# BGU-CS-VIL/DPMMSubClusters.jl

Measured on AMD Instinct MI355X. Metric: Gibbs iterations/sec, N=10M D=64 NIW, higher is better.
Workload: dtype f32

## Files before the change

### dpmmsubclusters.jl_amd/binding.py

```python
import ctypes
import os
import subprocess

import numpy as np

_HERE = os.path.dirname(os.path.abspath(__file__))
PRIOR_NIW, PRIOR_MULT = 0, 1
MAX_CLUSTERS = 1024

_c_i64p = ctypes.POINTER(ctypes.c_int64)
_c_f32p = ctypes.POINTER(ctypes.c_float)
_c_f64p = ctypes.POINTER(ctypes.c_double)

ABI = [
    ("dpmm_abi_version", ctypes.c_int, []),
    ("dpmm_create", ctypes.c_int, [ctypes.POINTER(ctypes.c_void_p), ctypes.c_int, ctypes.c_int, ctypes.c_int64, ctypes.c_int64, ctypes.c_int, ctypes.c_uint64]),
    ("dpmm_destroy", ctypes.c_int, [ctypes.c_void_p]),
    ("dpmm_last_error", ctypes.c_char_p, [ctypes.c_void_p]),
    ("dpmm_upload_points", ctypes.c_int, [ctypes.c_void_p, _c_f32p, ctypes.c_int64]),
    ("dpmm_upload_points_device", ctypes.c_int, [ctypes.c_void_p, ctypes.c_void_p, ctypes.c_int64]),
    ("dpmm_upload_points_npy", ctypes.c_int, [ctypes.c_void_p, ctypes.c_void_p, ctypes.c_int, ctypes.c_int64, ctypes.c_int]),
    ("dpmm_init_labels", ctypes.c_int, [ctypes.c_void_p, ctypes.c_int, ctypes.c_uint32]),
    ("dpmm_set_labels", ctypes.c_int, [ctypes.c_void_p, _c_i64p, _c_i64p]),
    ("dpmm_get_labels", ctypes.c_int, [ctypes.c_void_p, _c_i64p, _c_i64p]),
# ... 44 lines not shown
    ("dpmm_smart_assign", ctypes.c_int, [ctypes.c_void_p, ctypes.c_int64, ctypes.c_double, ctypes.c_double]),
    ("dpmm_debug_loglik", ctypes.c_int, [ctypes.c_void_p, _c_f32p]),
    ("dpmm_sync", ctypes.c_int, [ctypes.c_void_p]),
    ("dpmm_stream", ctypes.c_void_p, [ctypes.c_void_p]),
    ("dpmm_last_sweep_parts_ms", ctypes.c_int, [ctypes.c_void_p, _c_f32p]),
    ("dpmm_last_kernel_ms", ctypes.c_int, [ctypes.c_void_p, _c_f32p, _c_f32p]),
    ("dpmm_debug_counters", ctypes.c_int, [ctypes.c_void_p, ctypes.POINTER(ctypes.c_int64), ctypes.c_int]),
    ("dpmm_debug_set_prelaunch_hook", ctypes.c_int, [ctypes.c_void_p, ctypes.c_void_p]),
    ("dpmm_init_labels_from", ctypes.c_int, [ctypes.c_void_p, ctypes.c_int, ctypes.c_int, ctypes.c_uint32]),
    ("dpmm_set_option", ctypes.c_int, [ctypes.c_void_p, ctypes.c_int, ctypes.c_double]),
    ("dpmm_params_staging", ctypes.c_int, [ctypes.c_void_p, ctypes.c_int] + [ctypes.POINTER(ctypes.c_void_p)] * 6),
    ("dpmm_commit_params", ctypes.c_int, [ctypes.c_void_p, ctypes.c_int]),
    ("dpmm_suffstats_host", ctypes.c_int, [ctypes.c_void_p, _c_i64p, ctypes.c_int, ctypes.POINTER(ctypes.c_void_p)]),
    ("dpmm_step_stats", ctypes.c_int, [ctypes.c_void_p, ctypes.c_uint32, ctypes.POINTER(ctypes.c_void_p), ctypes.POINTER(ctypes.c_void_p)]),
    ("dpmm_debug_subloglik", ctypes.c_int, [ctypes.c_void_p, _c_f32p]),
    ("dpmm_debug_ref_bracket", ctypes.c_int, [ctypes.c_void_p, ctypes.c_int64, ctypes.c_float, _c_f32p, _c_f32p]),
    ("dpmm_debug_pair_ball", ctypes.c_int, [ctypes.c_void_p, _c_f32p, _c_f32p]),
    ("dpmm_debug_bracket_big", ctypes.c_int, [ctypes.c_void_p, _c_f32p, ctypes.POINTER(ctypes.c_uint32)]),
    ("dpmm_debug_mult_draws_ahead", ctypes.c_int, [ctypes.c_void_p, ctypes.POINTER(ctypes.c_longlong)]),
    ("dpmm_last_sweep_work", ctypes.c_int, [ctypes.c_void_p, ctypes.POINTER(ctypes.c_uint64)]),
    ("dpmm_comm_use_library", ctypes.c_int, [ctypes.c_char_p]),
    ("dpmm_comm_unique_id", ctypes.c_int, [ctypes.c_void_p]),
    ("dpmm_comm_init", ctypes.c_int, [ctypes.c_void_p, ctypes.c_void_p, ctypes.c_int, ctypes.c_int]),
    ("dpmm_comm_init_host", ctypes.c_int, [ctypes.c_void_p, ctypes.c_int, ctypes.c_int, ctypes.c_void_p, ctypes.c_void_p]),
    ("dpmm_comm_info", ctypes.c_int, [ctypes.c_void_p, _c_i64p]),
    ("dpmm_last_comm_ms", ctypes.c_int, [ctypes.c_void_p, _c_f32p, _c_f32p]),
    ("dpmm_comm_destroy", ctypes.c_int, [ctypes.c_void_p]),
    ("dpmm_comm_allgather_host", ctypes.c_int, [ctypes.c_void_p, ctypes.c_void_p, ctypes.c_int64, ctypes.c_void_p]),
]

HOST_ALLREDUCE_FN = ctypes.CFUNCTYPE(ctypes.c_int, ctypes.c_void_p, ctypes.c_void_p, ctypes.c_int64, ctypes.c_int)

MASTER_NSCALARS = 8
OPT_SCREEN_MARGIN, OPT_TAIL_SCREEN, OPT_PRESCREEN, OPT_ORDERED_SWEEP, OPT_MULT_FORCE_F32, OPT_STATS_ITEMS, OPT_STATS_GROUPS, OPT_TRACE_SLOW, OPT_LOGLIK_REF_CONST, OPT_WAVE_PRIO, OPT_MULT_NO_U8, OPT_SWEEP_GRID, OPT_SWEEP_QUEUE_ROUNDS, OPT_BALL_SCREEN, OPT_KERNEL_TIMING, OPT_STATS_DERIVE, OPT_NOISE_AHEAD, OPT_REF_BRACKET, OPT_SORT_TILE, OPT_ONE_COLLECTIVE, OPT_BF16_SCREENS, OPT_COMM_TIMEOUT_MS, OPT_DIRECTION_SCREEN, _OPT_RESERVED_24, OPT_MULT_DRAWS_AHEAD, OPT_B3_SUBLABELS, OPT_LEAN_TILES, OPT_MASTER_POLL, OPT_CHAIN_FUSION, OPT_LEAN_DIRECTION, OPT_PAIR_BALL = range(1, 32)


class DpmmError(RuntimeError):
    def __init__(self, code, msg):
        super().__init__(f"libdpmmhip error {code}: {msg}")
        self.code = code


def lib_path():
    return os.path.join(_HERE, "lib", "libdpmmhip.so")


def locked_make(args, lock_dir):
    import fcntl
    os.makedirs(lock_dir, exist_ok=True)
    with open(os.path.join(lock_dir, ".build.lock"), "w") as lk:
        fcntl.flock(lk, fcntl.LOCK_EX)
        try:
            subprocess.check_call(args)
        finally:
            fcntl.flock(lk, fcntl.LOCK_UN)


def build_library(force=False):
    args = ["make", "-s", "-C", os.path.join(_HERE, "csrc"), "-j4"]
    if force:
        args.append("-B")
    locked_make(args, os.path.join(_HERE, "lib"))
    return lib_path()


_LIB = None

# ... 482 lines not shown
```

### dpmmsubclusters.jl_amd/csrc/dpmm_api.cpp

```cpp
#include "../../include/dpmm_hip.h"
#include "../../include/dpmm_hip_master.h"
#include "../../include/dpmm_hip_debug.h"

#include <hip/hip_runtime.h>
#include <dlfcn.h>

#include <algorithm>
#include <atomic>
#include <condition_variable>
#include <mutex>
#include <thread>
#include <chrono>
#include <cmath>
#include <cstdio>
#include <cstring>
#include <cstdlib>
#include <ctime>
#include <string>
#include <unordered_map>
#include <vector>

#include "dpmm_kernels.h"

namespace dpmm {
// ... 157 lines not shown
    int32_t *h_list[4] = {nullptr, nullptr, nullptr, nullptr};
    size_t h_list_cap[4] = {0, 0, 0, 0};
    int h_list_next = 0;
    std::vector<int32_t> jobs_shadow, dslots_shadow;
    uint8_t *h_master = nullptr;
    size_t h_master_bytes = 0;
    bool draws_on_device = false;
    unsigned long long *d_work = nullptr;
    int work_waves = 0;
    long long work_launches = 0;
    float opt_margin = 50.f;
    int opt_prio = 1;
    int opt_queue_rounds = -1;
    int opt_ball = 1;
    uint32_t *d_sp_frag = nullptr;
    uint32_t *d_refb_big = nullptr;
    bool have_refb_big = false;
    uint32_t *d_brk_flag = nullptr;
    float *d_brk_aref = nullptr;
    float *d_sp_cons = nullptr;
    uint32_t *h_need = nullptr;
    int opt_direction = -1;
    bool sp_ready = false, sp_regime = false;
    unsigned sp_count = 0;
    bool sp_last = false;
    int sp_K = -1;
    int sp_cooldown = 0;
    int opt_b3 = 1;
    bool have_b3 = false;
    int opt_chain = 0x7fffffff & ~(8 | 32);
    int opt_pair_ball = 1;
    bool have_pb = false;
    int opt_lean_dir = 1;
    int opt_master_poll = 1;
    int opt_lean = 1;
    uint32_t *d_hard = nullptr;
    int hard_flip = 0;
    int perm_nbins = 0;
    uint32_t *h_hard = nullptr;
    int lean_off = 0;
    bool lean_ran = false;
    int lean_backoff = 15;
    int opt_bf16scr = 1;
    int opt_bracket = 1;
    int opt_timing = 0;
    int opt_tail = 1, opt_prescreen = -1, opt_ordered = 1, opt_force_f32 = 0, opt_trace = 0, opt_ref_const = 0;
    int64_t opt_stats_items = 0;
    int opt_stats_groups = 0;
    void *comm = nullptr;
    int rank = 0, world = 1;
    dpmm_host_allreduce_fn host_fn = nullptr;
    void *host_user = nullptr;
    char *h_red = nullptr;
    size_t h_red_bytes = 0;
    hipEvent_t ev_comm[4] = {nullptr, nullptr, nullptr, nullptr};
    bool have_comm_ev[2] = {false, false};
    int64_t comm_bytes[2] = {0, 0};
    int64_t comm_calls = 0;
    int comm_timeout_ms = 1800000;
    bool coll_pending = false;
    bool abort_reported = false;
    std::thread *watchdog = nullptr;
    std::mutex wd_mu;
    std::condition_variable wd_cv;
    bool wd_stop = false;
    std::atomic<int64_t> wd_wait_since{0};
// ... 868 lines not shown
            a.prio = c->opt_prio;
            a.queue_rounds = c->opt_queue_rounds;
        }
#ifdef DPMM_STAMPS
        if (!g_dbg) { hipMalloc(&g_dbg, sizeof(unsigned long long) * 16 * 4 * 4096); hipMemset(g_dbg, 0, sizeof(unsigned long long) * 16 * 4 * 4096); }
        a.dbg = g_dbg;
#endif
        const bool b3 = c->NB == 4 && c->have_b3 && c->opt_b3 && !table && !c->predictive && a.tail != nullptr;
        if (b3) {
            const bool lean_ok = c->opt_lean != 0 && c->opt_bracket && a.use_prev && a.screen_margin > 0.f && !final_argmax && a.lam == nullptr && c->K > 1 && c->d_hard &&
                                 !(c->opt_lean_dir == 0 && c->sp_regime && c->opt_direction != 0 && c->sp_ready);
            const int64_t nwt = (c->n + 63) / 64;
            if (lean_ok && c->lean_off == 0 && c->lean_ran) {
                if ((int64_t)c->h_hard[0] * 10 > nwt * 3) { c->lean_off = c->lean_backoff; c->lean_backoff = std::min(2 * c->lean_backoff + 1, 1023); }
                else c->lean_backoff = 15;
                c->lean_ran = false;
            }
            const bool use_lean = lean_ok && c->lean_off == 0;
            if (lean_ok && c->lean_off > 0) { c->lean_off -= 1; c->h_hard[0] = 0; }
            const uint32_t *list = nullptr;
            const bool parts = (c->opt_timing & 8) != 0 && (c->opt_timing & 1) != 0;
            if (parts && !c->ev_part[0]) for (auto &e : c->ev_part) HIPCHK(c, hipEventCreate(&e));
            if (use_lean) {
                const size_t hw = hard_list_words(c->n);
                uint32_t *mine = c->d_hard + (size_t)c->hard_flip * hw, *other = c->d_hard + (size_t)(c->hard_flip ^ 1) * hw;
                c->hard_flip ^= 1;
                c->lean_ran = true;
                uint32_t *need2 = a.need ? c->h_need + 8 * (size_t)c->sweep_grid_max : nullptr;
                const bool al = a.order != nullptr && c->perm_nbins > 0 && c->perm_nbins <= NIW_LEAN_MAX_BINS;
                uint32_t *need3 = a.need ? c->h_need + 12 * (size_t)c->sweep_grid_max : nullptr;
                NiwSweepArgs al_args = a;
                if (!c->opt_lean_dir) { al_args.sp_frag = nullptr; al_args.sp_cons = nullptr; }
                if (c->have_pb && c->opt_pair_ball && al_args.ball) al_args.ball |= 2;
                HIPCHK(c, launch_niw_lean(al_args, mine, need2, other, al ? c->sb.bin_start : nullptr, al ? c->perm_nbins : 0, need3, c->sweep_grid, c->stream));
                if (parts) HIPCHK(c, hipEventRecord(c->ev_part[0], c->stream));
                list = mine;
            }
            a.bf16scr |= 4;
            a.tdf = reinterpret_cast<const float *>(list);
            const float *mdist_kept = a.mdist;
            if (list) a.mdist = reinterpret_cast<const float *>(c->h_hard);
            HIPCHK(c, launch_niw_sweep(c->NB, a, c->sweep_grid, c->stream));
            a.mdist = mdist_kept;
            if (parts) HIPCHK(c, hipEventRecord(c->ev_part[1], c->stream));
            c->have_parts = parts ? (use_lean ? 2 : 1) : 0;
            a.bf16scr &= 3;
            a.tdf = nullptr;
            if (!list) HIPCHK(c, launch_niw_sub(a, nullptr, nullptr, c->sweep_grid, c->stream));
        } else {
            HIPCHK(c, launch_niw_sweep(c->NB, a, c->sweep_grid, c->stream));
            if (!table) c->have_parts = 0;
        }
    } else {
        MultSweepArgs a{};
        a.X = c->dX; a.ldx = c->ldx; a.n = c->n; a.first_index = c->first; a.D = c->D; a.K = c->K;
        a.logp = c->d_Rp; a.cst = c->d_cst;
        a.scratch = table ? table : c->d_scratch;
        a.scratch_stride = table ? table_stride : c->scratch_stride;
        a.scratch_by_tile = table ? 1 : 0;
        a.labels_only = table ? 1 : 0;
        a.bins = c->dbins; a.seed = c->seed; a.epoch = epoch; a.final_argmax = final_argmax;
        a.use_prev = c->have_labels ? 1 : 0;
        a.order = (!table && c->have_perm && c->opt_ordered) ? c->sb.perm : nullptr;
        a.order_total = c->sb.perm_total;
        if (c->x_u8) HIPCHK(c, launch_mult_sweep_u8(a, c->dX8, c->ld8, c->d_Lp16, c->sweep_grid, c->stream));
        else if (c->x_bf16_exact) HIPCHK(c, launch_mult_sweep_bf16(a, c->d_Lp16, c->sweep_grid, c->stream));
        else {
// ... 1286 lines not shown
}
#endif

void *dpmm_stream(dpmm_ctx *c) { return c ? (void *)c->stream : nullptr; }

int dpmm_set_option(dpmm_ctx *c, int option, double value) {
    if (!c) return DPMM_EINVAL;
    switch (option) {
        case DPMM_OPT_SCREEN_MARGIN: if (!(value >= 0)) return fail(c, DPMM_EINVAL, "margin < 0"); c->opt_margin = (float)value; return DPMM_OK;
        case DPMM_OPT_TAIL_SCREEN: c->opt_tail = value != 0; return DPMM_OK;
        case DPMM_OPT_PRESCREEN: c->opt_prescreen = value < 0 ? -1 : (value != 0); return DPMM_OK;
        case DPMM_OPT_ORDERED_SWEEP: c->opt_ordered = value != 0; return DPMM_OK;
        case DPMM_OPT_MULT_FORCE_F32:
            if (c->have_points) return fail(c, DPMM_ESTATE, "DPMM_OPT_MULT_FORCE_F32 must be set before the points are uploaded");
            c->opt_force_f32 = value != 0; return DPMM_OK;
        case DPMM_OPT_STATS_ITEMS:
            if (c->Kcap > 0) return fail(c, DPMM_ESTATE, "DPMM_OPT_STATS_ITEMS must be set before the first parameters / K");
            if (value >= 1) c->chunk = (int)std::max<int64_t>((c->prior == DPMM_PRIOR_NIW && c->D <= 64) ? 32 : 256, ((c->n + (int64_t)value - 1) / (int64_t)value + 3) / 4 * 4);
            return DPMM_OK;
        case DPMM_OPT_STATS_GROUPS: c->opt_stats_groups = value > 0 ? (int)value : 0; return DPMM_OK;
        case DPMM_OPT_TRACE_SLOW: c->opt_trace = value != 0; return DPMM_OK;
        case DPMM_OPT_LOGLIK_REF_CONST: c->opt_ref_const = value != 0; return DPMM_OK;
        case DPMM_OPT_WAVE_PRIO: c->opt_prio = value != 0; return DPMM_OK;
        case DPMM_OPT_MULT_DRAWS_AHEAD: c->opt_mult_draws_ahead = value != 0; c->mspec_valid = false; return DPMM_OK;
        case DPMM_OPT_SWEEP_QUEUE_ROUNDS: c->opt_queue_rounds = value < 0 ? -1 : (int)value; return DPMM_OK;
        case DPMM_OPT_BALL_SCREEN: c->opt_ball = value != 0; return DPMM_OK;
        case DPMM_OPT_STATS_DERIVE: c->opt_derive = value != 0; c->cache_force = true; return DPMM_OK;
        case DPMM_OPT_NOISE_AHEAD: c->opt_noise_ahead = value < 0 ? -1 : (value != 0); return DPMM_OK;
        case DPMM_OPT_REF_BRACKET: c->opt_bracket = value != 0; return DPMM_OK;
        case DPMM_OPT_COMM_TIMEOUT_MS: c->comm_timeout_ms = value > 0 ? (int)std::min(value, 2.0e9) : 0; return DPMM_OK;
        case DPMM_OPT_BF16_SCREENS: c->opt_bf16scr = value != 0; return DPMM_OK;
        case DPMM_OPT_MASTER_POLL: c->opt_master_poll = value != 0; return DPMM_OK;
        case DPMM_OPT_PAIR_BALL: c->opt_pair_ball = value != 0; if (!c->opt_pair_ball) c->have_pb = false; return DPMM_OK;
        case DPMM_OPT_LEAN_DIRECTION: c->opt_lean_dir = value != 0; c->lean_off = 0; c->lean_backoff = 15; c->lean_ran = false; return DPMM_OK;
        case DPMM_OPT_CHAIN_FUSION: c->opt_chain = value < 0 ? (0x7fffffff & ~(8 | 32)) : (int)value; return DPMM_OK;
        case DPMM_OPT_LEAN_TILES: c->opt_lean = value != 0; c->lean_off = 0; c->lean_backoff = 15; c->lean_ran = false; return DPMM_OK;
        case DPMM_OPT_B3_SUBLABELS: c->opt_b3 = value != 0; if (!c->opt_b3) c->have_b3 = false; return DPMM_OK;
        case DPMM_OPT_DIRECTION_SCREEN:
            c->opt_direction = value < 0 ? -1 : (value != 0);
            if (c->opt_direction == 0) { c->sp_ready = false; c->sp_regime = false; }
            return DPMM_OK;
        case DPMM_OPT_ONE_COLLECTIVE: c->opt_one_collective = value < 0 ? -1 : (value != 0); return DPMM_OK;
        case DPMM_OPT_SORT_TILE: {
            const int t = (int)value;
            if (t != SORT_TILE && t != SORT_TILE_SMALL) return fail(c, DPMM_EINVAL, "DPMM_OPT_SORT_TILE: 512 or 2048");
            if (t < c->sort_tile_min) {
                if (c->n > 16000000) return fail(c, DPMM_ELIMIT, "DPMM_OPT_SORT_TILE: 512-point tiles are limited to shards of 16e6 points");
                HIPCHK(c, hipSetDevice(c->device));
                HIPCHK(c, sync_stream(c, c->stream));
                const int nt = (int)((c->n + t - 1) / t);
                const size_t nbmax = 2 * DPMM_MAX_CLUSTERS;
                int32_t *th = nullptr, *tc = nullptr, *tsp = nullptr;
                HIPCHK(c, hipMalloc(&th, sizeof(int32_t) * nbmax * (size_t)std::max(1, nt)));
                if (hipMalloc(&tc, sizeof(int32_t) * nbmax * (size_t)std::max(1, nt)) != hipSuccess) { hipFree(th); return fail(c, DPMM_EHIP, "DPMM_OPT_SORT_TILE: out of device memory for the 512-point tile tables"); }
                if (hipMalloc(&tsp, sizeof(int32_t) * (size_t)STEP_SPEC_MAX_BINS * (size_t)std::max(1, nt)) != hipSuccess) { hipFree(th); hipFree(tc); return fail(c, DPMM_EHIP, "DPMM_OPT_SORT_TILE: out of device memory for the 512-point tile tables"); }
                hipFree(c->sb.tile_hist); hipFree(c->sb.tile_cnt); hipFree(c->sb.tile_spec);
                c->sb.tile_hist = th; c->sb.tile_cnt = tc; c->sb.tile_spec = tsp;
                c->nt_sort = nt; c->sort_tile_min = t;
            }
            c->sb.tile = t; return DPMM_OK;
        }
        case DPMM_OPT_KERNEL_TIMING:
            c->opt_timing = (int)value & 15;
            if (!(c->opt_timing & 1)) c->have_sweep_ev = false;
            if (!(c->opt_timing & 2)) c->have_stats_ev = false;
            if (!(c->opt_timing & 4)) c->have_comm_ev[0] = c->have_comm_ev[1] = false;
// ... 302 lines not shown
```

### dpmmsubclusters.jl_amd/csrc/dpmm_kernels.h

```cpp
#pragma once
#include <hip/hip_runtime.h>
#include <stdint.h>

#define DPMM_MAX_CLUSTERS_K 1024

namespace dpmm {


constexpr int DPMM_WORK_QUEUES = 8;
constexpr int DPMM_WORK_SLOTS = 8 + 16 * DPMM_WORK_QUEUES;
constexpr int DPMM_WORK_PER_WAVE = 8;
constexpr int REFB_FRAGS = 6, REFB_WORDS = REFB_FRAGS * 256;
constexpr int B3_WORDS = 3 * REFB_WORDS;
constexpr int B3_DVEC = 64;

struct NiwSweepArgs {
    const float *X;
    int64_t ldx;
    int64_t n;
    int64_t first_index;
    int64_t ntiles;
    int K;
    const float *Rp;
    const float *mup;
// ... 19 lines not shown
    const float *mdist;
    int screen_lds;
    int use_prev;
    int lds_rows;
    const uint32_t *sp_frag;
    const float *sp_cons;
    uint32_t *need;
    unsigned long long *dbg;
    int queue_rounds;
    int prio;
    unsigned long long *work;
};

int niw_tile_points(int NB);
int niw_occupancy(int NB);
hipError_t launch_niw_sweep(int NB, const NiwSweepArgs &a, int grid, hipStream_t s);
hipError_t launch_niw_refb_debug(const NiwSweepArgs &a, int k, float c_override, float *qhi_out, float *q_out, hipStream_t s);
hipError_t launch_niw_screen_prep(const float *R, const float *mu, int D, int K, float *lam, float *dist, const int32_t *slot, hipStream_t s);
hipError_t launch_niw_pack(const float *R, const float *mu, float *Rp, float *mup, int D, int NB, int nmat, float *tail, const float *cst,
                           const int32_t *slot, float *cst_out, unsigned long long *work, hipStream_t s);
constexpr int SP_MAXK = 64, SP_FRAG_WORDS = 4 * 2 * 256, SP_CONS_FLOATS = 3 * 64;
inline size_t niw_refb_big_words(int NB) { size_t c = 0; for (int bi = 0; bi < NB; ++bi) c += NB / 2 - bi / 2; return c * 256; }
hipError_t launch_niw_refb_big(const float *Rp, int NB, int K, uint32_t *out, hipStream_t s);
hipError_t launch_niw_bracket_big(int NB, const NiwSweepArgs &a, const uint32_t *refb, uint32_t *tile_flag, float *aref, hipStream_t s);
hipError_t launch_niw_b3_pack(const float *Rp, const float *mup, int K, float *tail, int what, hipStream_t s);
constexpr int PB_MAXK = 256;
inline size_t niw_pair_ball_floats(size_t K) { return K <= (size_t)PB_MAXK ? K * K + K : 0; }
inline size_t niw_pair_ball_offset(size_t K) { return 32 * ((K + 1) >> 1) + 16 * K + (size_t)REFB_WORDS * K + 3 * K * (size_t)B3_WORDS + 3 * K * (size_t)B3_DVEC; }
inline size_t niw_tail_floats(size_t cap) {
    return 16 * (cap + 2) + 16 * cap + (size_t)REFB_WORDS * cap + 3 * cap * (size_t)B3_WORDS + 3 * cap * (size_t)B3_DVEC + niw_pair_ball_floats(cap < (size_t)PB_MAXK ? cap : (size_t)PB_MAXK);
}
hipError_t launch_niw_b3_debug(const NiwSweepArgs &a, float *out, hipStream_t s);
hipError_t launch_niw_sub(const NiwSweepArgs &a, const uint32_t *list, uint32_t *count_out, int grid, hipStream_t s);
constexpr int NIW_LEAN_MAX_BINS = 256;
hipError_t launch_niw_lean(const NiwSweepArgs &a, uint32_t *list, uint32_t *need2, uint32_t *other_list, const int32_t *bin_start, int nbins, uint32_t *need3, int grid, hipStream_t s);
hipError_t launch_niw_direction(const float *Rp, const float *mup, const float *cst, int D, int K, uint32_t *frag, float *cons, hipStream_t s);

struct MultSweepArgs {
    const float *X;
    int64_t ldx;
    int64_t n;
    int64_t first_index;
    int D;
    int K;
    const float *logp;
    const float *cst;
    float *scratch;
    int64_t scratch_stride;
    int scratch_by_tile;
    int labels_only;
    int32_t *bins;
    uint64_t seed;
    uint32_t epoch;
    int final_argmax;
    int use_prev;
    const int32_t *order;
    const int32_t *order_total;
};
hipError_t launch_mult_sweep(const MultSweepArgs &a, int grid, hipStream_t s);
hipError_t launch_mult_pack(const float *logp, float *Lp, int rows, int64_t ldx, hipStream_t s);
int mult_tile_points();
hipError_t launch_bf16_exact_check(const float *X, int64_t nwords, int *d_flag, hipStream_t s);
size_t mult_pack_bf16_words(int rows, int64_t ldx);
hipError_t launch_mult_pack_bf16(const float *logp, uint32_t *Lp16, int rows, int64_t ldx, hipStream_t s);
hipError_t launch_mult_sweep_bf16(const MultSweepArgs &a, const uint32_t *Lp16, int grid, hipStream_t s);
hipError_t launch_u8_convert(const float *X, int64_t ldx, int D, int64_t n, uint8_t *X8, int64_t ld8, int *d_flag, hipStream_t s);
size_t mult_pack_u8_words(int rows, int64_t ld8);
hipError_t launch_mult_pack_u8(const float *logp, uint32_t *Lp8, int rows, int64_t ldx, int64_t ld8, hipStream_t s);
// ... 142 lines not shown
```

### dpmmsubclusters.jl_amd/csrc/niw_lean.hip

```cpp
#include "dpmm_device.h"
#include "dpmm_kernels.h"
#include "niw_device.h"
#include "niw_b3.h"

namespace dpmm {

__global__ __launch_bounds__(256) void niw_b3_pack_kernel(const float *__restrict__ Rp, const float *__restrict__ mup, float *__restrict__ tail, int K, int y0) {
    constexpr int NP = 10;
    uint32_t *img = const_cast<uint32_t *>(b3_images(tail, K));
    float *dvec = const_cast<float *>(b3_offsets(tail, K));
    const int k = blockIdx.x >> 1, j = 3 * k + 1 + (blockIdx.x & 1);
    const float *Rj = Rp + (size_t)j * NP * 256;
    auto elem = [&](int row, int col) -> float {
        const int bi = row >> 4, t = col >> 4;
        if (t < bi) return 0.f;
        const int pair = pair_base<4>(bi) + (t - bi);
        const int ln = (row & 15) + 16 * ((col & 15) >> 2);
        return Rj[(size_t)pair * 256 + ln * 4 + (col & 3)];
    };
    const int yy = (int)blockIdx.y + y0;
    if (yy == 4) {
        if (blockIdx.x & 1) return;
        const float *Rk = Rp + (size_t)(3 * k) * NP * 256;
        auto elemR = [&](int row, int col) -> float {
// ... 145 lines not shown
#pragma unroll
            for (int sl = 0; sl < 2; ++sl) {
                const int f = bi == 0 ? sl : (bi == 1 ? 2 + sl : (sl == 1 ? bi + 2 : -1));
                if (f < 0) continue;
                const u32x4_t aa = a[f] & absm;
#pragma unroll
                for (int h = 0; h < 2; ++h) {
                    const u32x4_t zb = Z.p[n0 + h][sl][0];
                    y[h] = __builtin_amdgcn_mfma_f32_16x16x32_bf16(__builtin_bit_cast(bf16x8_t, a[f]), __builtin_bit_cast(bf16x8_t, zb), y[h], 0, 0, 0);
                    e[h] = __builtin_amdgcn_mfma_f32_16x16x32_bf16(__builtin_bit_cast(bf16x8_t, aa), __builtin_bit_cast(bf16x8_t, zb & absm), e[h], 0, 0, 0);
                }
            }
#pragma unroll
            for (int h = 0; h < 2; ++h)
#pragma unroll
                for (int r = 0; r < 4; ++r) {
                    const float t = __builtin_fmaf(REFB_C, e[h][r], fabsf(y[h][r]));
                    part[h] = __builtin_fmaf(t, t, part[h]);
                }
        }
#pragma unroll
        for (int h = 0; h < 2; ++h) {
            const f32x4 tot = __builtin_amdgcn_mfma_f32_16x16x4f32(1.0f, part[h], (f32x4){0.f, 0.f, 0.f, 0.f}, 0, 0, 0);
            qhi[n0 + h] = __builtin_fmaf(tot[0], 1.0001f, 1e-20f);
        }
    }
}

#ifdef DPMM_STAMPS
#define LSTAMP(var) unsigned long long var; do { __builtin_amdgcn_sched_barrier(0); asm volatile("s_memtime %0\n\ts_waitcnt lgkmcnt(0)" : "=s"(var) :: "memory"); __builtin_amdgcn_sched_barrier(0); } while (0)
#else
#define LSTAMP(var)
#endif
template <bool DIR>
__device__ __forceinline__ void niw_lean_body(NiwSweepArgs A, uint32_t *__restrict__ list, uint32_t *__restrict__ need2, uint32_t *__restrict__ other_list,
                                              const int32_t *__restrict__ bin_start, int nbins, uint32_t *__restrict__ need3) {
    if (other_list && blockIdx.x == 0 && threadIdx.x == 0) other_list[0] = 0u;
#ifdef DPMM_STAMPS
    unsigned long long T_x = 0, T_conv = 0, T_br = 0, T_scr = 0, T_u = 0, T_p2 = 0, T_tot = 0; int ntl = 0;
#endif
    const int lane = threadIdx.x & 63, ci = lane & 15, g = lane >> 4;
    const bool use_order = A.order != nullptr && *A.order_total == (int32_t)A.n;
    const int K = A.K;
    const int wave_id = (int)blockIdx.x * 4 + (threadIdx.x >> 6), nwaves = (int)gridDim.x * 4;
    unsigned nw_easy = 0, nw_br = 0, nw_tail = 0, nw_bb = 0;
    const bool use_dir = DIR && A.sp_frag != nullptr && A.sp_cons != nullptr && A.bf16scr && K >= 3 && K <= SP_MAXK;
    const bool dir_first = use_dir && (A.bf16scr & 2) != 0;
    unsigned nw_sp = 0, nw_cand = 0, nw_dcand = 0, nw_dexcl = 0, nw_ctiles = 0;
    constexpr int BALL_LDS_K = 256;
    __shared__ __attribute__((aligned(16))) float ball_lds[BALL_LDS_K * 16];
    const bool ball_in_lds = A.ball && K <= BALL_LDS_K;
    __shared__ float pb_s[PB_MAXK];
    const bool use_pb = !DIR && (A.ball & 2) != 0 && ball_in_lds && K <= PB_MAXK;
    const float *pb_d = pair_ball_table(A.tail, K);
    if (use_pb)
        for (int e = threadIdx.x; e < K; e += 256) pb_s[e] = pb_d[(size_t)K * K + e];
    if (ball_in_lds) {
        const float *src = ball_records(A.tail, K);
        for (int e = threadIdx.x; e < 16 * K; e += 256) ball_lds[e] = src[e];
    }
    constexpr int MAXB = NIW_LEAN_MAX_BINS;
    __shared__ int tstart_s[MAXB + 2], bstart_s[MAXB + 2], wsum_s[4];
    const bool aligned = bin_start != nullptr && use_order && nbins >= 1 && nbins <= MAXB && bin_start[nbins] == (int32_t)A.n;
    const int nb = aligned ? nbins : 1;
    {
        const int tid = threadIdx.x;
        int c = 0;
        if (tid < nb) {
            const int s0 = aligned ? bin_start[tid] : 0, s1 = aligned ? bin_start[tid + 1] : (int)A.n;
            c = (s1 - s0 + 63) >> 6; bstart_s[tid] = s0;
        }
        if (tid == 0) bstart_s[nb] = (int)A.n;
        int inc = c;
#pragma unroll
        for (int off = 1; off < 64; off <<= 1) { const int v = __shfl_up(inc, off); if (lane >= off) inc += v; }
        if (lane == 63) wsum_s[tid >> 6] = inc;
        __syncthreads();
        const int w = tid >> 6;
        inc += (w > 0 ? wsum_s[0] : 0) + (w > 1 ? wsum_s[1] : 0) + (w > 2 ? wsum_s[2] : 0);
        tstart_s[tid + 1] = inc;
        if (tid == 0) tstart_s[0] = 0;
    }
    __syncthreads();
    const int ntiles_all = __builtin_amdgcn_readfirstlane(tstart_s[nb]);
    int bptr = 0;
    auto span_of = [&](int t, int &p0, int &cn) {
        p0 = 0; cn = 0;
        if (t >= ntiles_all) return;
        while (t >= __builtin_amdgcn_readfirstlane(tstart_s[bptr + 1])) ++bptr;
        p0 = __builtin_amdgcn_readfirstlane(bstart_s[bptr]) + 64 * (t - __builtin_amdgcn_readfirstlane(tstart_s[bptr]));
        const int e = __builtin_amdgcn_readfirstlane(bstart_s[bptr + 1]) - p0;
        cn = e < 64 ? e : 64;
    };
    auto index_at = [&](int p0, int cn) -> int { return lane < cn ? (use_order ? A.order[p0 + lane] : p0 + lane) : -1; };
    int c_p0, c_cn, n_p0, n_cn;
    span_of(wave_id, c_p0, c_cn);
    span_of(wave_id + nwaves, n_p0, n_cn);
    int nx_p = index_at(c_p0, c_cn);
    auto label_of = [&](int bin) -> int { const int pv = bin >= 0 ? (bin >> 1) : -1; return (unsigned)pv < (unsigned)K ? pv : -1; };
    int nx_prev = label_of(nx_p >= 0 ? A.bins[nx_p] : -1);
    for (int tile = wave_id; tile < ntiles_all; tile += nwaves) {
        const bool valid = lane < c_cn;
        const int myp32 = nx_p;
        LSTAMP(s0);
#ifdef DPMM_STAMPS
        unsigned long long s1 = s0, s2 = s0, s3 = s0, s4 = s0, s5 = s0;
#endif
        const int pf_p = index_at(n_p0, n_cn);
        int pf_bin = -1;
        bool bin_asked = false;
        const int prev = nx_prev;
        const unsigned long long pm = __ballot(prev >= 0);
        bool hard = pm == 0ull;
        int k0 = 0;
        if (!hard) {
            k0 = __builtin_amdgcn_readfirstlane(__shfl(prev, __ffsll((long long)pm) - 1));
            hard = __ballot(valid && prev != k0) != 0ull;
        }
        B3Z Z;
        B3Head H;
        float u_sub = 0.f;
        if (!hard) {
            f32x4 xt = (f32x4){0.f, 0.f, 0.f, 0.f};
            f32x4 x3[4];
            float nz[4] = {0.f, 0.f, 0.f, 0.f};
            u32x4_t abr[6];
            {
                f32x4 x[4][4], mk[4];
                gather_x64(A.X, A.ldx, myp32, ci, g, x);
                b3_mean(A.mup, k0, g, mk);
                {
                    const u32x4_t *F = reinterpret_cast<const u32x4_t *>(refb_records(A.tail, K) + (size_t)k0 * REFB_WORDS) + (unsigned)lane;
#pragma unroll
                    for (int f = 0; f < 6; ++f) abr[f] = F[64 * f];
// ... 102 lines not shown
                    const int pr = (base + sh) >> 1;
                    pend &= ~(3ull << sh);
                    ++nw_tail;
                    cand &= ~((unsigned long long)tail_pair_far(tail_load_pair(A.tail, pr), xt, my_thr) << sh);
                }
                if constexpr (DIR) { if (use_dir && !dir_first) { tile_cand = (unsigned)__builtin_popcountll(cand); direction(); } }
                if (A.bf16scr) {
                    const u32x4_t *Rb0 = reinterpret_cast<const u32x4_t *>(refb_records(A.tail, K));
                    while (cand) {
                        const int k = base + __builtin_ctzll(cand);
                        const u32x4_t a5 = Rb0[(size_t)k * (REFB_WORDS / 4) + 64 * 5 + lane];
                        const f32x4 m4 = *reinterpret_cast<const f32x4 *>(A.mup + (size_t)(3 * k) * 64 + 48 + 4 * g);
                        ++nw_bb;
                        if (!bf16_bottom_excludes<4>(a5, x3, m4, A.cst[3 * k], thrb)) break;
                        cand &= cand - 1ull;
                    }
                }
                hard = cand != 0ull;
                if constexpr (DIR) { if (use_dir && !hard) { nw_cand += tile_cand; nw_sp += tile_sp; nw_dcand += tile_dc; nw_dexcl += tile_dx; ++nw_ctiles; } }
            }
        }
#ifdef DPMM_STAMPS
        { LSTAMP(t4); s4 = t4; }
#endif
        if (!hard) {
            H = b3_head(A.tail, A.cst, K, k0, lane, g);
        }
#ifdef DPMM_STAMPS
        { LSTAMP(t5); s5 = t5; }
#endif
        if (hard) {
            if (lane == 0) { const uint32_t at = atomicAdd(&list[0], 1u); list[1 + 2 * at] = (uint32_t)c_p0; list[2 + 2 * at] = (uint32_t)c_cn; }
            if (!bin_asked && lane < n_cn) pf_bin = A.bins[pf_p];
        } else {
            float bl, br;
            b3_eval(A.tail, K, k0, Z, H, lane, g, bl, br);
            if (valid) A.bins[myp32] = 2 * k0 + draw2(bl, br, u_sub);
            ++nw_easy;
        }
        nx_p = pf_p; nx_prev = label_of(pf_bin);
        asm volatile("" : "+v"(nx_prev));
        c_p0 = n_p0; c_cn = n_cn;
        span_of(tile + 2 * nwaves, n_p0, n_cn);
#ifdef DPMM_STAMPS
        { LSTAMP(s6); T_x += s1 - s0; T_conv += s2 - s1; T_br += s3 - s2; T_scr += s4 - s3; T_u += s5 - s4; T_p2 += s6 - s5; T_tot += s6 - s0; ++ntl; }
#endif
    }
#ifdef DPMM_STAMPS
    if (A.dbg && lane == 0) {
        unsigned long long *d = A.dbg + (size_t)(8192 + wave_id) * 16;
        d[0] = T_x; d[1] = T_conv; d[2] = T_br; d[3] = T_scr; d[4] = T_u; d[5] = T_p2; d[6] = 0; d[7] = T_tot; d[8] = ntl;
    }
#endif
    if (A.work && lane == 0) {
        unsigned long long *slot = A.work + DPMM_WORK_SLOTS + (size_t)wave_id * DPMM_WORK_PER_WAVE;
        slot[0] += nw_easy; slot[3] += nw_tail; slot[4] += nw_br; slot[5] += nw_bb; slot[7] += ((unsigned long long)(2 * nw_easy) << 32) + nw_sp;
    }
    if (need2 && lane == 0) need2[wave_id] = use_dir ? 0u : (nw_easy < 65535u ? nw_easy : 65535u);
    if (need3 && lane == 0) {
        uint32_t word = 0u, yield = 0u;
        if (use_dir) {
            word = ((nw_cand < 65535u ? nw_cand : 65535u) << 16) | (nw_ctiles < 32767u ? nw_ctiles : 32767u) | (dir_first ? 0x8000u : 0u);
            yield = ((nw_dexcl < 65535u ? nw_dexcl : 65535u) << 16) | (nw_dcand < 65535u ? nw_dcand : 65535u);
        }
        need3[2 * wave_id] = word; need3[2 * wave_id + 1] = yield;
    }
}
__global__ __launch_bounds__(256, 2) void niw_lean_kernel(NiwSweepArgs A, uint32_t *__restrict__ list, uint32_t *__restrict__ need2, uint32_t *__restrict__ other_list,
                                                         const int32_t *__restrict__ bin_start, int nbins, uint32_t *__restrict__ need3) {
    niw_lean_body<false>(A, list, need2, other_list, bin_start, nbins, need3);
}
__global__ __launch_bounds__(256, 2) void niw_lean_kernel_dir(NiwSweepArgs A, uint32_t *__restrict__ list, uint32_t *__restrict__ need2, uint32_t *__restrict__ other_list,
                                                             const int32_t *__restrict__ bin_start, int nbins, uint32_t *__restrict__ need3) {
    niw_lean_body<true>(A, list, need2, other_list, bin_start, nbins, need3);
}
hipError_t launch_niw_lean(const NiwSweepArgs &a, uint32_t *list, uint32_t *need2, uint32_t *other_list, const int32_t *bin_start, int nbins, uint32_t *need3, int grid, hipStream_t s) {
    if (!a.tail || a.n <= 0 || !list) return hipErrorInvalidValue;
    if (nbins > NIW_LEAN_MAX_BINS) { bin_start = nullptr; nbins = 0; }
    if (a.sp_frag && a.sp_cons && a.bf16scr && a.K >= 3 && a.K <= SP_MAXK) DPMM_LAUNCH(niw_lean_kernel_dir, dim3(grid), dim3(256), 0, s, a, list, need2, other_list, bin_start, nbins, need3);
    else DPMM_LAUNCH(niw_lean_kernel, dim3(grid), dim3(256), 0, s, a, list, need2, other_list, bin_start, nbins, need3);
    return hipGetLastError();
}

}
```

### include/dpmm_hip.h

```cpp
#ifndef DPMM_HIP_H
#define DPMM_HIP_H

#include <stddef.h>
#include <stdint.h>

#ifdef __cplusplus
extern "C" {
#endif

#define DPMM_ABI_VERSION 3

typedef struct dpmm_ctx dpmm_ctx;

enum { DPMM_PRIOR_NIW = 0, DPMM_PRIOR_MULT = 1 };

enum {
    DPMM_OK = 0,
    DPMM_EINVAL = -1,
    DPMM_ENODEVICE = -2,
    DPMM_EHIP = -3,
    DPMM_ESTATE = -4,
    DPMM_ELIMIT = -5,
    DPMM_ECOMM = -6
};

enum {
    DPMM_OPT_SCREEN_MARGIN = 1,
    DPMM_OPT_TAIL_SCREEN = 2,
    DPMM_OPT_PRESCREEN = 3,
    DPMM_OPT_ORDERED_SWEEP = 4,
    DPMM_OPT_MULT_FORCE_F32 = 5,
    DPMM_OPT_STATS_ITEMS = 6,
    DPMM_OPT_STATS_GROUPS = 7,
    DPMM_OPT_TRACE_SLOW = 8,
    DPMM_OPT_LOGLIK_REF_CONST = 9,
    DPMM_OPT_MULT_NO_U8 = 11,
    DPMM_OPT_SWEEP_GRID = 12,
    DPMM_OPT_SWEEP_QUEUE_ROUNDS = 13,
    DPMM_OPT_BALL_SCREEN = 14,
    DPMM_OPT_STATS_DERIVE = 16,
    DPMM_OPT_NOISE_AHEAD = 17,
    DPMM_OPT_REF_BRACKET = 18,
    DPMM_OPT_SORT_TILE = 19,
    DPMM_OPT_COMM_TIMEOUT_MS = 22,
    DPMM_OPT_B3_SUBLABELS = 26,
    DPMM_OPT_LEAN_TILES = 27,
    DPMM_OPT_MASTER_POLL = 28,
    DPMM_OPT_CHAIN_FUSION = 29,
    DPMM_OPT_LEAN_DIRECTION = 30,
    DPMM_OPT_PAIR_BALL = 31,
    DPMM_OPT_MULT_DRAWS_AHEAD = 25,
    DPMM_OPT_DIRECTION_SCREEN = 23,
    DPMM_OPT_BF16_SCREENS = 21,
    DPMM_OPT_ONE_COLLECTIVE = 20,
    DPMM_OPT_KERNEL_TIMING = 15,
    DPMM_OPT_WAVE_PRIO = 10
};

#define DPMM_MAX_CLUSTERS 1024
#define DPMM_MAX_DIM_NIW 256

int dpmm_abi_version(void);

int dpmm_create(dpmm_ctx **ctx, int prior_kind, int D, int64_t n_local, int64_t first_index,
                int device, uint64_t seed);
int dpmm_destroy(dpmm_ctx *ctx);
const char *dpmm_last_error(const dpmm_ctx *ctx);

int dpmm_upload_points(dpmm_ctx *ctx, const float *X, int64_t ldx);
int dpmm_upload_points_device(dpmm_ctx *ctx, const float *dX, int64_t ldx);
int dpmm_upload_points_npy(dpmm_ctx *ctx, const void *rows, int is_f64, int64_t ld, int nan_to_zero);

int dpmm_init_labels(dpmm_ctx *ctx, int init_clusters, uint32_t epoch);
int dpmm_init_labels_from(dpmm_ctx *ctx, int init_clusters, int first_label, uint32_t epoch);
int dpmm_set_option(dpmm_ctx *ctx, int option, double value);
int dpmm_set_labels(dpmm_ctx *ctx, const int64_t *labels, const int64_t *sub_labels);
int dpmm_get_labels(dpmm_ctx *ctx, int64_t *labels, int64_t *sub_labels);

int dpmm_set_params_niw(dpmm_ctx *ctx, int K, const float *mu, const float *inv_sigma, const float *logdet,
                        const float *lr_weights, const float *weights);
int dpmm_set_params_niw_chol(dpmm_ctx *ctx, int K, const float *mu, const float *R, const float *logdet,
                             const float *lr_weights, const float *weights);
int dpmm_set_params_mult(dpmm_ctx *ctx, int K, const float *logp, const float *lr_weights, const float *weights);
// ... 57 lines not shown
```

Baseline: 696.2.

## Pair waves in 512-thread lean blocks with staggered start and token-gated b3 eval

Adds a paired variant of the lean NIW sweep kernel in which each 512-thread block hosts two groups of four waves. The second group runs at raised priority, waits for its partner to finish a tile before starting, and both groups take turns through a shared-memory token around the b3_eval section. The goal is to stagger phases so one wave's compute overlaps its partner's memory latency and they don't contend for the same unit. It is on by default for the non-direction path (pairing=1), while the direction kernel needs pairing=2. Bounded spin-polls with s_sleep add latency and can stall if the pairing is imbalanced.

Measured after the change: 705.3 (median of 6 runs). 1.01x the previous value.

```diff
diff --git a/dpmmsubclusters.jl_amd/binding.py b/dpmmsubclusters.jl_amd/binding.py
--- a/dpmmsubclusters.jl_amd/binding.py
+++ b/dpmmsubclusters.jl_amd/binding.py
@@ -100,7 +100,7 @@
 HOST_ALLREDUCE_FN = ctypes.CFUNCTYPE(ctypes.c_int, ctypes.c_void_p, ctypes.c_void_p, ctypes.c_int64, ctypes.c_int)
 
 MASTER_NSCALARS = 8
-OPT_SCREEN_MARGIN, OPT_TAIL_SCREEN, OPT_PRESCREEN, OPT_ORDERED_SWEEP, OPT_MULT_FORCE_F32, OPT_STATS_ITEMS, OPT_STATS_GROUPS, OPT_TRACE_SLOW, OPT_LOGLIK_REF_CONST, OPT_WAVE_PRIO, OPT_MULT_NO_U8, OPT_SWEEP_GRID, OPT_SWEEP_QUEUE_ROUNDS, OPT_BALL_SCREEN, OPT_KERNEL_TIMING, OPT_STATS_DERIVE, OPT_NOISE_AHEAD, OPT_REF_BRACKET, OPT_SORT_TILE, OPT_ONE_COLLECTIVE, OPT_BF16_SCREENS, OPT_COMM_TIMEOUT_MS, OPT_DIRECTION_SCREEN, _OPT_RESERVED_24, OPT_MULT_DRAWS_AHEAD, OPT_B3_SUBLABELS, OPT_LEAN_TILES, OPT_MASTER_POLL, OPT_CHAIN_FUSION, OPT_LEAN_DIRECTION, OPT_PAIR_BALL = range(1, 32)
+OPT_SCREEN_MARGIN, OPT_TAIL_SCREEN, OPT_PRESCREEN, OPT_ORDERED_SWEEP, OPT_MULT_FORCE_F32, OPT_STATS_ITEMS, OPT_STATS_GROUPS, OPT_TRACE_SLOW, OPT_LOGLIK_REF_CONST, OPT_WAVE_PRIO, OPT_MULT_NO_U8, OPT_SWEEP_GRID, OPT_SWEEP_QUEUE_ROUNDS, OPT_BALL_SCREEN, OPT_KERNEL_TIMING, OPT_STATS_DERIVE, OPT_NOISE_AHEAD, OPT_REF_BRACKET, OPT_SORT_TILE, OPT_ONE_COLLECTIVE, OPT_BF16_SCREENS, OPT_COMM_TIMEOUT_MS, OPT_DIRECTION_SCREEN, _OPT_RESERVED_24, OPT_MULT_DRAWS_AHEAD, OPT_B3_SUBLABELS, OPT_LEAN_TILES, OPT_MASTER_POLL, OPT_CHAIN_FUSION, OPT_LEAN_DIRECTION, OPT_PAIR_BALL, OPT_LEAN_PAIRING = range(1, 33)
 
 
 class DpmmError(RuntimeError):
diff --git a/dpmmsubclusters.jl_amd/csrc/dpmm_api.cpp b/dpmmsubclusters.jl_amd/csrc/dpmm_api.cpp
--- a/dpmmsubclusters.jl_amd/csrc/dpmm_api.cpp
+++ b/dpmmsubclusters.jl_amd/csrc/dpmm_api.cpp
@@ -213,6 +213,7 @@
     int opt_pair_ball = 1;
     bool have_pb = false;
     int opt_lean_dir = 1;
+    int opt_lean_pair = DPMM_LEAN_PAIRING_DEFAULT;
     int opt_master_poll = 1;
     int opt_lean = 1;
     uint32_t *d_hard = nullptr;
@@ -1147,7 +1148,7 @@
                 NiwSweepArgs al_args = a;
                 if (!c->opt_lean_dir) { al_args.sp_frag = nullptr; al_args.sp_cons = nullptr; }
                 if (c->have_pb && c->opt_pair_ball && al_args.ball) al_args.ball |= 2;
-                HIPCHK(c, launch_niw_lean(al_args, mine, need2, other, al ? c->sb.bin_start : nullptr, al ? c->perm_nbins : 0, need3, c->sweep_grid, c->stream));
+                HIPCHK(c, launch_niw_lean(al_args, mine, need2, other, al ? c->sb.bin_start : nullptr, al ? c->perm_nbins : 0, need3, c->sweep_grid, c->opt_lean_pair, c->stream));
                 if (parts) HIPCHK(c, hipEventRecord(c->ev_part[0], c->stream));
                 list = mine;
             }
@@ -2500,6 +2501,7 @@
         case DPMM_OPT_BF16_SCREENS: c->opt_bf16scr = value != 0; return DPMM_OK;
         case DPMM_OPT_MASTER_POLL: c->opt_master_poll = value != 0; return DPMM_OK;
         case DPMM_OPT_PAIR_BALL: c->opt_pair_ball = value != 0; if (!c->opt_pair_ball) c->have_pb = false; return DPMM_OK;
+        case DPMM_OPT_LEAN_PAIRING: c->opt_lean_pair = value < 0 ? DPMM_LEAN_PAIRING_DEFAULT : std::min((int)value, 2); return DPMM_OK;
         case DPMM_OPT_LEAN_DIRECTION: c->opt_lean_dir = value != 0; c->lean_off = 0; c->lean_backoff = 15; c->lean_ran = false; return DPMM_OK;
         case DPMM_OPT_CHAIN_FUSION: c->opt_chain = value < 0 ? (0x7fffffff & ~(8 | 32)) : (int)value; return DPMM_OK;
         case DPMM_OPT_LEAN_TILES: c->opt_lean = value != 0; c->lean_off = 0; c->lean_backoff = 15; c->lean_ran = false; return DPMM_OK;
diff --git a/dpmmsubclusters.jl_amd/csrc/dpmm_kernels.h b/dpmmsubclusters.jl_amd/csrc/dpmm_kernels.h
--- a/dpmmsubclusters.jl_amd/csrc/dpmm_kernels.h
+++ b/dpmmsubclusters.jl_amd/csrc/dpmm_kernels.h
@@ -75,8 +75,9 @@
 }
 hipError_t launch_niw_b3_debug(const NiwSweepArgs &a, float *out, hipStream_t s);
 hipError_t launch_niw_sub(const NiwSweepArgs &a, const uint32_t *list, uint32_t *count_out, int grid, hipStream_t s);
+constexpr int DPMM_LEAN_PAIRING_DEFAULT = 1;
 constexpr int NIW_LEAN_MAX_BINS = 256;
-hipError_t launch_niw_lean(const NiwSweepArgs &a, uint32_t *list, uint32_t *need2, uint32_t *other_list, const int32_t *bin_start, int nbins, uint32_t *need3, int grid, hipStream_t s);
+hipError_t launch_niw_lean(const NiwSweepArgs &a, uint32_t *list, uint32_t *need2, uint32_t *other_list, const int32_t *bin_start, int nbins, uint32_t *need3, int grid, int pair, hipStream_t s);
 hipError_t launch_niw_direction(const float *Rp, const float *mup, const float *cst, int D, int K, uint32_t *frag, float *cons, hipStream_t s);
 
 struct MultSweepArgs {
diff --git a/dpmmsubclusters.jl_amd/csrc/niw_lean.hip b/dpmmsubclusters.jl_amd/csrc/niw_lean.hip
--- a/dpmmsubclusters.jl_amd/csrc/niw_lean.hip
+++ b/dpmmsubclusters.jl_amd/csrc/niw_lean.hip
@@ -201,9 +201,13 @@
 #else
 #define LSTAMP(var)
 #endif
-template <bool DIR>
+constexpr int LEAN_STAGGER_POLLS = 192, LEAN_TOKEN_POLLS = 48;
+__device__ __forceinline__ int lean_pair_peek(int *w) { return __hip_atomic_load(w, __ATOMIC_RELAXED, __HIP_MEMORY_SCOPE_WORKGROUP); }
+__device__ __forceinline__ void lean_pair_post(int *w, int v) { __hip_atomic_store(w, v, __ATOMIC_RELAXED, __HIP_MEMORY_SCOPE_WORKGROUP); }
+template <bool DIR, bool PAIR>
 __device__ __forceinline__ void niw_lean_body(NiwSweepArgs A, uint32_t *__restrict__ list, uint32_t *__restrict__ need2, uint32_t *__restrict__ other_list,
-                                              const int32_t *__restrict__ bin_start, int nbins, uint32_t *__restrict__ need3) {
+                                              const int32_t *__restrict__ bin_start, int nbins, uint32_t *__restrict__ need3, int pair_nwaves = 0) {
+    constexpr int NT = PAIR ? 512 : 256, NWV = NT / 64;
     if (other_list && blockIdx.x == 0 && threadIdx.x == 0) other_list[0] = 0u;
 #ifdef DPMM_STAMPS
     unsigned long long T_x = 0, T_conv = 0, T_br = 0, T_scr = 0, T_u = 0, T_p2 = 0, T_tot = 0; int ntl = 0;
@@ -211,7 +215,15 @@
     const int lane = threadIdx.x & 63, ci = lane & 15, g = lane >> 4;
     const bool use_order = A.order != nullptr && *A.order_total == (int32_t)A.n;
     const int K = A.K;
-    const int wave_id = (int)blockIdx.x * 4 + (threadIdx.x >> 6), nwaves = (int)gridDim.x * 4;
+    const int wv = __builtin_amdgcn_readfirstlane((int)(threadIdx.x >> 6));
+    const int wave_id = (int)blockIdx.x * NWV + wv, nwaves = PAIR ? pair_nwaves : (int)gridDim.x * 4;
+    const bool has_slot = !PAIR || wave_id < nwaves;
+    __shared__ int pair_s[PAIR ? 16 : 1];
+    const bool younger = PAIR && wv >= 4;
+    if constexpr (PAIR) {
+        if (threadIdx.x < 16) pair_s[threadIdx.x] = 0;
+        if (younger) __builtin_amdgcn_s_setprio(1);
+    }
     unsigned nw_easy = 0, nw_br = 0, nw_tail = 0, nw_bb = 0;
     const bool use_dir = DIR && A.sp_frag != nullptr && A.sp_cons != nullptr && A.bf16scr && K >= 3 && K <= SP_MAXK;
     const bool dir_first = use_dir && (A.bf16scr & 2) != 0;
@@ -223,13 +235,13 @@
     const bool use_pb = !DIR && (A.ball & 2) != 0 && ball_in_lds && K <= PB_MAXK;
     const float *pb_d = pair_ball_table(A.tail, K);
     if (use_pb)
-        for (int e = threadIdx.x; e < K; e += 256) pb_s[e] = pb_d[(size_t)K * K + e];
+        for (int e = threadIdx.x; e < K; e += NT) pb_s[e] = pb_d[(size_t)K * K + e];
     if (ball_in_lds) {
         const float *src = ball_records(A.tail, K);
-        for (int e = threadIdx.x; e < 16 * K; e += 256) ball_lds[e] = src[e];
+        for (int e = threadIdx.x; e < 16 * K; e += NT) ball_lds[e] = src[e];
     }
     constexpr int MAXB = NIW_LEAN_MAX_BINS;
-    __shared__ int tstart_s[MAXB + 2], bstart_s[MAXB + 2], wsum_s[4];
+    __shared__ int tstart_s[MAXB + 2], bstart_s[MAXB + 2], wsum_s[NWV];
     const bool aligned = bin_start != nullptr && use_order && nbins >= 1 && nbins <= MAXB && bin_start[nbins] == (int32_t)A.n;
     const int nb = aligned ? nbins : 1;
     {
@@ -247,11 +259,15 @@
         __syncthreads();
         const int w = tid >> 6;
         inc += (w > 0 ? wsum_s[0] : 0) + (w > 1 ? wsum_s[1] : 0) + (w > 2 ? wsum_s[2] : 0);
-        tstart_s[tid + 1] = inc;
+        if (!PAIR || tid < 256) tstart_s[tid + 1] = inc;
         if (tid == 0) tstart_s[0] = 0;
     }
     __syncthreads();
     const int ntiles_all = __builtin_amdgcn_readfirstlane(tstart_s[nb]);
+    if constexpr (PAIR) {
+        if (younger && has_slot && wave_id < ntiles_all)
+            for (int i = 0; i < LEAN_STAGGER_POLLS && __builtin_amdgcn_readfirstlane(lean_pair_peek(&pair_s[8 + (wv & 3)])) == 0; ++i) __builtin_amdgcn_s_sleep(4);
+    }
     int bptr = 0;
     auto span_of = [&](int t, int &p0, int &cn) {
         p0 = 0; cn = 0;
@@ -263,12 +279,13 @@
     };
     auto index_at = [&](int p0, int cn) -> int { return lane < cn ? (use_order ? A.order[p0 + lane] : p0 + lane) : -1; };
     int c_p0, c_cn, n_p0, n_cn;
-    span_of(wave_id, c_p0, c_cn);
-    span_of(wave_id + nwaves, n_p0, n_cn);
+    const int tile0 = has_slot ? wave_id : ntiles_all;
+    span_of(tile0, c_p0, c_cn);
+    span_of(has_slot ? wave_id + nwaves : ntiles_all, n_p0, n_cn);
     int nx_p = index_at(c_p0, c_cn);
     auto label_of = [&](int bin) -> int { const int pv = bin >= 0 ? (bin >> 1) : -1; return (unsigned)pv < (unsigned)K ? pv : -1; };
     int nx_prev = label_of(nx_p >= 0 ? A.bins[nx_p] : -1);
-    for (int tile = wave_id; tile < ntiles_all; tile += nwaves) {
+    for (int tile = tile0; tile < ntiles_all; tile += nwaves) {
         const bool valid = lane < c_cn;
         const int myp32 = nx_p;
         LSTAMP(s0);
@@ -437,9 +454,17 @@
         if (hard) {
             if (lane == 0) { const uint32_t at = atomicAdd(&list[0], 1u); list[1 + 2 * at] = (uint32_t)c_p0; list[2 + 2 * at] = (uint32_t)c_cn; }
             if (!bin_asked && lane < n_cn) pf_bin = A.bins[pf_p];
+            if constexpr (PAIR) lean_pair_post(&pair_s[8 + wv], 1);
         } else {
+            if constexpr (PAIR) {
+                lean_pair_post(&pair_s[8 + wv], 1);
+                for (int i = 0; i < LEAN_TOKEN_POLLS && __builtin_amdgcn_readfirstlane(lean_pair_peek(&pair_s[wv ^ 4])) != 0; ++i) __builtin_amdgcn_s_sleep(4);
+                lean_pair_post(&pair_s[wv], 1);
+                __builtin_amdgcn_sched_barrier(0);
+            }
             float bl, br;
             b3_eval(A.tail, K, k0, Z, H, lane, g, bl, br);
+            if constexpr (PAIR) { __builtin_amdgcn_sched_barrier(0); lean_pair_post(&pair_s[wv], 0); }
             if (valid) A.bins[myp32] = 2 * k0 + draw2(bl, br, u_sub);
             ++nw_easy;
         }
@@ -451,10 +476,17 @@
         { LSTAMP(s6); T_x += s1 - s0; T_conv += s2 - s1; T_br += s3 - s2; T_scr += s4 - s3; T_u += s5 - s4; T_p2 += s6 - s5; T_tot += s6 - s0; ++ntl; }
 #endif
     }
+    if constexpr (PAIR) {
+        lean_pair_post(&pair_s[8 + wv], 1);
+        if (!has_slot) return;
+    }
 #ifdef DPMM_STAMPS
     if (A.dbg && lane == 0) {
         unsigned long long *d = A.dbg + (size_t)(8192 + wave_id) * 16;
         d[0] = T_x; d[1] = T_conv; d[2] = T_br; d[3] = T_scr; d[4] = T_u; d[5] = T_p2; d[6] = 0; d[7] = T_tot; d[8] = ntl;
+        unsigned hwid;
+        asm volatile("s_getreg_b32 %0, hwreg(HW_REG_HW_ID)" : "=s"(hwid));
+        d[9] = hwid; d[10] = (unsigned long long)blockIdx.x * 8 + (threadIdx.x >> 6);
     }
 #endif
     if (A.work && lane == 0) {
@@ -473,16 +505,29 @@
 }
 __global__ __launch_bounds__(256, 2) void niw_lean_kernel(NiwSweepArgs A, uint32_t *__restrict__ list, uint32_t *__restrict__ need2, uint32_t *__restrict__ other_list,
                                                          const int32_t *__restrict__ bin_start, int nbins, uint32_t *__restrict__ need3) {
-    niw_lean_body<false>(A, list, need2, other_list, bin_start, nbins, need3);
+    niw_lean_body<false, false>(A, list, need2, other_list, bin_start, nbins, need3);
 }
 __global__ __launch_bounds__(256, 2) void niw_lean_kernel_dir(NiwSweepArgs A, uint32_t *__restrict__ list, uint32_t *__restrict__ need2, uint32_t *__restrict__ other_list,
                                                              const int32_t *__restrict__ bin_start, int nbins, uint32_t *__restrict__ need3) {
-    niw_lean_body<true>(A, list, need2, other_list, bin_start, nbins, need3);
-}
-hipError_t launch_niw_lean(const NiwSweepArgs &a, uint32_t *list, uint32_t *need2, uint32_t *other_list, const int32_t *bin_start, int nbins, uint32_t *need3, int grid, hipStream_t s) {
-    if (!a.tail || a.n <= 0 || !list) return hipErrorInvalidValue;
+    niw_lean_body<true, false>(A, list, need2, other_list, bin_start, nbins, need3);
+}
+__global__ __launch_bounds__(512) void niw_lean_pair_kernel(NiwSweepArgs A, uint32_t *__restrict__ list, uint32_t *__restrict__ need2, uint32_t *__restrict__ other_list,
+                                                            const int32_t *__restrict__ bin_start, int nbins, uint32_t *__restrict__ need3, int pair_nwaves) {
+    niw_lean_body<false, true>(A, list, need2, other_list, bin_start, nbins, need3, pair_nwaves);
+}
+__global__ __launch_bounds__(512) void niw_lean_pair_kernel_dir(NiwSweepArgs A, uint32_t *__restrict__ list, uint32_t *__restrict__ need2, uint32_t *__restrict__ other_list,
+                                                                const int32_t *__restrict__ bin_start, int nbins, uint32_t *__restrict__ need3, int pair_nwaves) {
+    niw_lean_body<true, true>(A, list, need2, other_list, bin_start, nbins, need3, pair_nwaves);
+}
+hipError_t launch_niw_lean(const NiwSweepArgs &a, uint32_t *list, uint32_t *need2, uint32_t *other_list, const int32_t *bin_start, int nbins, uint32_t *need3, int grid, int pair, hipStream_t s) {
+    if (!a.tail || a.n <= 0 || !list || grid < 1) return hipErrorInvalidValue;
     if (nbins > NIW_LEAN_MAX_BINS) { bin_start = nullptr; nbins = 0; }
-    if (a.sp_frag && a.sp_cons && a.bf16scr && a.K >= 3 && a.K <= SP_MAXK) DPMM_LAUNCH(niw_lean_kernel_dir, dim3(grid), dim3(256), 0, s, a, list, need2, other_list, bin_start, nbins, need3);
+    const bool dir = a.sp_frag && a.sp_cons && a.bf16scr && a.K >= 3 && a.K <= SP_MAXK;
+    if (pair >= (dir ? 2 : 1)) {
+        const int g2 = (grid + 1) / 2, nw = 4 * grid;
+        if (dir) DPMM_LAUNCH(niw_lean_pair_kernel_dir, dim3(g2), dim3(512), 0, s, a, list, need2, other_list, bin_start, nbins, need3, nw);
+        else DPMM_LAUNCH(niw_lean_pair_kernel, dim3(g2), dim3(512), 0, s, a, list, need2, other_list, bin_start, nbins, need3, nw);
+    } else if (dir) DPMM_LAUNCH(niw_lean_kernel_dir, dim3(grid), dim3(256), 0, s, a, list, need2, other_list, bin_start, nbins, need3);
     else DPMM_LAUNCH(niw_lean_kernel, dim3(grid), dim3(256), 0, s, a, list, need2, other_list, bin_start, nbins, need3);
     return hipGetLastError();
 }
diff --git a/include/dpmm_hip.h b/include/dpmm_hip.h
--- a/include/dpmm_hip.h
+++ b/include/dpmm_hip.h
@@ -49,6 +49,7 @@
     DPMM_OPT_CHAIN_FUSION = 29,
     DPMM_OPT_LEAN_DIRECTION = 30,
     DPMM_OPT_PAIR_BALL = 31,
+    DPMM_OPT_LEAN_PAIRING = 32,
     DPMM_OPT_MULT_DRAWS_AHEAD = 25,
     DPMM_OPT_DIRECTION_SCREEN = 23,
     DPMM_OPT_BF16_SCREENS = 21,
```
